# obeychoi0120/wseg

Measured on AMD Instinct MI355X. Metric: training images/sec at B=16x448x448 (contrast_train step), higher is better.
Workload: dtype bf16; 1 GPU; ResNet-38 contrast, synthetic VOC 448x448, B=16/GPU, procedural weights, dropout on, fused HIP loss; global_batch=16, parallelism=dp1, seed=0

## Files before the change

include/wseg_hip.h:

```cpp
#ifndef WSEG_HIP_H
#define WSEG_HIP_H
#include <stddef.h>
#include <stdint.h>
#ifdef __cplusplus
extern "C" {
#endif

#define WSEG_F32 0
#define WSEG_BF16 1
#define WSEG_F32X3 2

int wseg_version(void);
size_t wseg_sizeof_conv_desc(void);
size_t wseg_sizeof_wgrad_desc(void);
const char* wseg_last_error(void);

typedef struct wseg_conv_desc {
  const void* in;  const void* w;  void* out;  void* out2;
  const void* r_pre;  const void* r_post;  const void* mask;
  const float* scale;  const float* shift;  const float* drop;
  int32_t N, IH, IW, IC, ld_in;
  int32_t OH, OW, OC, ld_out, ld_out2;
  int32_t ld_rpre, ld_rpost, ld_mask;
  int32_t KH, KW, stride, dil, pad;
  int32_t mode, epi, dtype;
  int32_t relu_out2;
  int32_t relu_lt;
  int32_t bm_hint;
  int32_t IH2, IW2, OH2, OW2;
  const void* in2;
  int32_t ld_in2, IC2;
  int32_t w_rows;
} wseg_conv_desc;
int wseg_conv_igemm(const wseg_conv_desc* d, void* stream);

typedef struct wseg_wgrad_desc {
  const void* x;  const void* dy;  float* dw;
  int32_t N, IH, IW, IC, ld_x;
  int32_t OH, OW, OC, ld_dy;
  int32_t KH, KW, stride, dil, pad;
  int32_t dtype, split_k;
  int32_t IC_dw, OC_dw;
  int32_t tile_hint;
  int32_t IH2, IW2, OH2, OW2;
  int32_t dw_rot;
} wseg_wgrad_desc;
int wseg_conv_wgrad(const wseg_wgrad_desc* d, void* stream);

#define WSEG_CONV_64x128 1
#define WSEG_CONV_128x128 2
#define WSEG_CONV_224x256 3
#define WSEG_CONV_256x256 4
#define WSEG_CONV_512x128 5
#define WSEG_WGRAD_128x128 6
#define WSEG_WGRAD_256x256 7
typedef struct wseg_launch_plan {
  int32_t family;
  int32_t tile_rows, tile_cols;
  int32_t nwg;
  int32_t perm;
  int32_t tapf;
  int32_t nsplit;
  int32_t unit;
} wseg_launch_plan;
int wseg_conv_plan(const wseg_conv_desc* d, wseg_launch_plan* out);
int wseg_wgrad_plan(const wseg_wgrad_desc* d, wseg_launch_plan* out);

int wseg_conv_bwd_pair(const wseg_conv_desc* dg, const wseg_wgrad_desc* wg, void* stream);
int wseg_conv_bwd_pair_plan(const wseg_conv_desc* dg, const wseg_wgrad_desc* wg, wseg_launch_plan* dg_plan, wseg_launch_plan* wg_plan);

int wseg_pack_weights(const float* master, void* fwd, void* tr, int OC, int T, int IC,
                      int OCp, int ICp, int ic_rot, int dtype, void* stream);
int wseg_copy2d_batch(const void* src, void* dst, const long* table, int npieces, long total_chunks, void* stream);
int wseg_pack_transposed_batch(const float* master, void* out, const long* table, int nlayers, long total_tiles, int dtype, void* stream);
int wseg_pack_transposed_batch_bf16(const void* mirror, void* out, const long* table, int nlayers, long total_tiles, void* stream);
int wseg_dropout_scale(const float* u, float* out, long total, long split_at, float p0, float p1, void* stream);

int wseg_stem_conv(const float* x_nchw, const float* w ,
                   const float* scale, const float* shift, void* raw, void* act,
                   int N, int H, int W, int dtype, void* stream);
int wseg_stem_conv_kc(const float* x, const float* w_kc, const float* scale, const float* shift,
                      void* raw, void* act, int N, int H, int W, int dtype, void* stream);

int wseg_head_split(const void* head, int ld, int c0, float* cam_low, float* cmax, int N, int hw, int dtype, void* stream);
int wseg_cam_gate(const float* cam_low, const float* cmax, float* G, int N, int hw, void* stream);
int wseg_pcm_xs(const float* x_nchw, void* feat, int ld, int c_xs, int c_end, int N, int H, int W, int h, int w, int dtype, void* stream);
int wseg_head_grad_rows(const float* d_fproj, const float* d_cam_low, const void* head, void* d_head, int ld, int N, int hw, int dtype, void* stream);

int wseg_resize_planar_fwd(const float* in, float* out, const float* plane_mul, long planes, int ih, int iw, int oh, int ow, int align,
                           int flip_x, int accumulate, void* stream);
int wseg_resize_planar_bwd(const float* d_out, float* d_in, const float* plane_mul, const float* plane_add, long planes, int ih, int iw, int oh, int ow, int align, int accumulate, void* stream);

int wseg_infer_finish(const float* sum_cam, const float* stats, float alpha, float* norm_cam, unsigned char* pred, int npix, void* stream);

int wseg_l2norm_forward(const void* F, int ldf, float* Fh, float* nrm, long rows, int dtype, void* stream);
int wseg_l2norm_backward(const void* F, int ldf, const float* dFh, const float* nrm, void* dF, int lddf, long rows, int dtype, void* stream);
int wseg_pcm_forward(const float* Fh, const float* G, float* cam_rv, float* den, int N, int hw, void* stream);
int wseg_pcm_backward(const float* Fh, const float* G, const float* d_cam_rv, const float* cam_rv, const float* den,
                      float* DN, float* dFh, int N, int hw, void* stream);
int wseg_pack_x3(const float* src, void* dst, long numel, void* stream);
int wseg_split_bf16(const float* in, void* hi, void* lo, long total, void* stream);
int wseg_to_bf16(const float* in, void* out, long total, void* stream);
int wseg_pcm_forward_bf16(const void* Fb, const void* Gb, float* cam_rv, float* den, int N, int hw, void* stream);
int wseg_pcm_backward_bf16(const void* Fb, const void* Gb, const void* Gl, const float* d_cam_rv, const float* cam_rv, const float* den,
                           float* DN, void* DNb, void* DNl, float* dFh, int N, int hw, void* stream);

size_t wseg_plane_stats_workspace_bytes(long planes);
int wseg_plane_stats(const float* U, float* stats, long planes, int npix, void* workspace, void* stream);
int wseg_up_plane_stats(const float* low, float* stats, long planes, int h, int w, int S, const float* label20 , void* workspace, void* stream);
int wseg_up_rvmin_values(const float* low, const float* label20, float* q, unsigned char* argc, int N, int h, int w, int S, void* stream);
int wseg_up_norm_resize_forward(const float* low, const float* stats, const float* label20, float* out, int N, int h, int w, int S, int OS, void* stream);
int wseg_resize_adjoint_ones(float* wvec, int h, int S, void* stream);
int wseg_up_maps_backward(const float* G, const float* low, const float* stats, const float* label20, const float* plane_bias,
                          const float* wvec_y, const float* wvec_x, const float* q, const unsigned char* argc, const float* res,
                          int k, float coef, float* d_low, int N, int h, int w, int S, int OS, void* stream);
int wseg_cls_loss(const float* stats, const float* label20, float* loss_out, float* plane_bias, int N, int npix, float coef, void* stream);
size_t wseg_select_workspace_bytes(int rows);
int wseg_select_kth(const float* vals, int rows, int n, int k, int largest, int use_abs, int relu_vals, float* res, void* workspace, void* stream);
int wseg_select_finish(const float* res, int rows, int k, int relu_vals, float scale, float* loss_out, void* stream);
int wseg_loss_finish(const float* acc, float er_coef, float* out8, void* stream);
int wseg_er_ecr_prep(const float* c1, const float* c2, const float* r1, const float* r2, float* Gc1, float* Gc2, float* dlt1, float* dlt2,
                     float* er_sum, int N, int npix, float er_coef, void* stream);
int wseg_ecr_backward(const float* dlt, const float* res, float* Gr, int N, int per_row, int k, float coef, void* stream);
int wseg_rows_resize_forward(const void* head, int ld, float* F, int N, int ih, int iw, int oh, int ow, int dtype, void* stream);
int wseg_head_grad_fused(const float* dF, const float* d_cam_low, const void* head, void* d_head, int ld, int N, int ih, int iw, int oh, int ow, int dtype, void* stream);
int wseg_pseudo_label(const float* R, const float* label20, float bg_thr, int* y, float* ncam, int N, int npix, void* stream);
int wseg_proto_candidates(const float* ncam, const float* F, const int* tie_idx, float* cand_val, float* cand_feat, int* cand_const, int N, int npix, int K, void* stream);
int wseg_proto_merge(const float* cand_val, const float* cand_feat, const int* cand_const, float* protos, int world, int K,
                     long rank_stride , void* stream);
int wseg_intra_weights(const int* y, const float* S_own, int ld_s, const float* rkey, const unsigned char* rand_flag, float* w, int P, void* stream);
int wseg_intra_weights_global(const float* rec, float* w, int P, int ranks, int own_rank, float scale, long rank_stride, void* stream);

typedef struct {
  const float* F;
  const float* p_own;
  const float* p_oth;
  const int32_t* y_own;
  const int32_t* y_oth;
  const float* w_intra;
  const float* rkey;
  float* rec;
  float* dF;
} wseg_nce_view;
int wseg_nce_records(const wseg_nce_view* views, int nviews, int P, int split_bf16, void* stream);
int wseg_nce_fused(const wseg_nce_view* views, int nviews, int P, float coef_cross, float coef_intra, float* sums , void* stream);

typedef struct {
  const uint8_t* src; int32_t H, W;
  int32_t rh, rw;
  const int32_t* xb; const int32_t* xk; int32_t xks;
  const int32_t* yb; const int32_t* yk; int32_t yks;
  uint8_t* tmp; uint8_t* img;
  int32_t flip;
  int32_t op[4];
  float factor[4];
  int32_t hue_shift;
  int32_t cont_top, cont_left, img_top, img_left, ch, cw;
  float* out;
} wseg_aug_desc;
size_t wseg_sizeof_aug_desc(void);
int wseg_augment_batch(const wseg_aug_desc* descs_dev, int n, int max_pixels , const float* lut ,
                       int crop, unsigned long long* lum_sums , void* stream);

int wseg_sgd_step(float* params, const float* grads, float* momentum_buf, long numel,
                  const long* seg_begin, const long* seg_end, const float* seg_lr, const float* seg_wd, int nseg,
                  float momentum, float grad_scale, int first_step, void* bf16_mirror, void* stream);

#define WSEG_AFF_MAX_OFFSETS 64
#define WSEG_RW_MAX_PLANE 8192
int wseg_aff_num_offsets(int radius);
int wseg_aff_pairs(const void* feat, int ld, int C, float* aff, int N, int h, int w, int radius, int dtype, void* stream);
int wseg_aff_to_dense(const float* aff, float* dense, int h, int w, int radius, void* stream);
int wseg_rw_prepare(const float* aff, float* wgt, float* rsum, int N, int h, int w, int radius, int beta, void* stream);
int wseg_random_walk(const float* wgt, const float* rsum, const float* v_in, float* v_out, int N, int planes, int h, int w, int radius,
                     int logt, void* stream);
int wseg_rw_pool(const float* cams, const int* src, float bg, float* pooled, int H, int W, int dh, int dw, void* stream);
int wseg_rw_finish(const float* cam_rw, unsigned char* pred, int planes, int dh, int dw, int H, int W, void* stream);

long wseg_aff_loss_workspace_bytes(int N, int h, int w, int radius);
int wseg_aff_loss_forward(const void* feat, int ld, int C, const unsigned char* label, float* aff, void* workspace, float* out7, int N,
                          int h, int w, int radius, int dtype, void* stream);
int wseg_aff_loss_backward(const void* feat, int ld, int C, const unsigned char* label, const float* aff, const float* out7,
                           const float* gscale, float* d_feat, int ld_d, int N, int h, int w, int radius, int dtype, void* stream);

int wseg_elu_backward_rows(const void* g, int ld_g, int g_dtype, const void* y, int ld_y, int y_dtype, const float* gscale, void* dz,
                           int ld_dz, int dz_dtype, long M, int C, void* stream);

#define WSEG_CRF_PIX_ALIGN 128
// ... 21 lines not shown
```

wseg_amd/_lib.py:

```python
import contextlib
import ctypes as C
import os

import torch

_HERE = os.path.dirname(os.path.abspath(__file__))
LIB_PATH = os.environ.get("WSEG_LIB") or os.path.join(_HERE, "libwseg_hip.so")

F32, BF16, F32X3 = 0, 1, 2
PROFILE_WGRAD = None
PROFILE = None
PROFILE_STRIDE = 1
_profile_idx = 0
_profile_phase = 0


def profile_begin_step(step):
    global _profile_idx, _profile_phase
    _profile_idx, _profile_phase = 0, step % max(1, PROFILE_STRIDE)


def _profile_sample():
    global _profile_idx
    i = _profile_idx
# ... 20 lines not shown
    _fields_ = [("x", C.c_void_p), ("dy", C.c_void_p), ("dw", C.c_void_p),
                ("N", C.c_int32), ("IH", C.c_int32), ("IW", C.c_int32), ("IC", C.c_int32), ("ld_x", C.c_int32),
                ("OH", C.c_int32), ("OW", C.c_int32), ("OC", C.c_int32), ("ld_dy", C.c_int32),
                ("KH", C.c_int32), ("KW", C.c_int32), ("stride", C.c_int32), ("dil", C.c_int32), ("pad", C.c_int32),
                ("dtype", C.c_int32), ("split_k", C.c_int32), ("IC_dw", C.c_int32), ("OC_dw", C.c_int32),
                ("tile_hint", C.c_int32),
                ("IH2", C.c_int32), ("IW2", C.c_int32), ("OH2", C.c_int32), ("OW2", C.c_int32), ("dw_rot", C.c_int32)]


def _load():
    if not os.path.exists(LIB_PATH):
        raise ImportError(
            f"{LIB_PATH} not found: build it with `python -c 'import __graft_entry__ as g; g.build()'` "
            "(wseg_amd has no CPU/eager fallback)")
    lib = C.CDLL(LIB_PATH)
    lib.wseg_last_error.restype = C.c_char_p
    lib.wseg_version.restype = C.c_int
    for fn in ("wseg_sizeof_conv_desc", "wseg_sizeof_wgrad_desc", "wseg_select_workspace_bytes", "wseg_plane_stats_workspace_bytes"):
        getattr(lib, fn).restype = C.c_size_t
    if lib.wseg_sizeof_conv_desc() != C.sizeof(ConvDesc) or lib.wseg_sizeof_wgrad_desc() != C.sizeof(WgradDesc):
        raise ImportError(f"{LIB_PATH} was built from another include/wseg_hip.h (descriptor sizes "
                          f"{lib.wseg_sizeof_conv_desc()}/{lib.wseg_sizeof_wgrad_desc()} vs {C.sizeof(ConvDesc)}/{C.sizeof(WgradDesc)}): rebuild it")
    return lib


lib = _load()


def _ptr(t):
    return t.data_ptr() if torch.is_tensor(t) else t


def stream_ptr():
    return torch.cuda.current_stream().cuda_stream


def check(status, what):
    if status != 0:
        raise RuntimeError(f"{what} failed ({status}): {lib.wseg_last_error().decode()}")


def _v(x):
    return C.c_void_p(_ptr(x))


def _s():
    return C.c_void_p(stream_ptr())


def _f(x):
    return C.c_float(x)


def _call(name, *args):
    check(getattr(lib, name)(*args, _s()), name)


def dtype_code(t):
    if t.dtype == torch.float32:
        return F32
    if t.dtype == torch.bfloat16:
        return BF16
    raise TypeError(f"unsupported dtype {t.dtype}")


def _flops_label(kind, *, N, IH, IW, IC, OH, OW, OC, KH, KW, stride=1, dil=1, seg2=None, mode=0, IC2=None, **_):
    oh, ow = (OH, OW) if mode == 0 else (IH, IW)
    pix = N * oh * ow
    if seg2 is not None:
        pix += N * (seg2[2] * seg2[3] if mode == 0 else seg2[0] * seg2[1])
    kin = IC * KH * KW + (IC2 or 0)
    return 2.0 * pix * kin * OC, f"{kind} {IC}{('+%d' % IC2) if IC2 else ''}->{OC} k{KH} s{stride} d{dil} {OH}x{OW}"


@contextlib.contextmanager
def _timed(sink, entry):
    if sink is None:
        yield
        return
    ev0, ev1 = torch.cuda.Event(enable_timing=True), torch.cuda.Event(enable_timing=True)
    ev0.record()
    yield
    ev1.record()
    sink.append((ev0, ev1) + tuple(entry()))


def conv_igemm(inp, w, out=None, out2=None, *, pair_wgrad=None, **kw):
    d = _conv_desc(inp, w, out, out2, **kw)
    ic2 = (d.IC2 or d.IC) if d.in2 else 0
    krow, wrows = d.KH * d.KW * d.IC + ic2, max(d.OC, d.w_rows)
    if w.numel() < wrows * krow:
        raise RuntimeError(f"conv_igemm: weight buffer has {w.numel()} elements, the launch reads {wrows} x {krow}")
    sampled, launch_idx = _profile_sample() if PROFILE is not None else (False, 0)

    def entry():
        kind = "fwd" if d.mode == 0 else ("dgrad+wgrad" if pair_wgrad is not None else "dgrad")
        flops, label = _flops_label(kind, **{**kw, "IC2": ic2})
        wflops = _flops_label("wgrad", **pair_wgrad[3])[0] if pair_wgrad is not None else 0.0
        return flops + wflops, label, launch_idx

    with _timed(PROFILE if sampled else None, entry):
        if pair_wgrad is not None:
            wx, wdy, wdw, wkw = pair_wgrad
            _call("wseg_conv_bwd_pair", C.byref(d), C.byref(_wgrad_desc(wx, wdy, wdw, **wkw)))
        else:
            _call("wseg_conv_igemm", C.byref(d))


def _conv_desc(inp, w, out, out2, *, N, IH, IW, IC, OH, OW, OC, KH, KW, stride=1, dil=1, pad=0,
               mode=0, epi=0, r_pre=None, r_post=None, mask=None, scale=None, shift=None, drop=None,
               ld_in=None, ld_out=None, ld_out2=None, ld_rpre=None, ld_rpost=None, ld_mask=None, relu_out2=1,
               relu_lt=0, bm_hint=0, seg2=None, in2=None, ld_in2=None, IC2=0, dtype=None, w_rows=0):
    d = ConvDesc()
    d.inp, d.w, d.out, d.out2 = _ptr(inp), _ptr(w), _ptr(out), _ptr(out2)
    d.r_pre, d.r_post, d.mask = _ptr(r_pre), _ptr(r_post), _ptr(mask)
    d.scale, d.shift, d.drop = _ptr(scale), _ptr(shift), _ptr(drop)
    d.N, d.IH, d.IW, d.IC, d.ld_in = N, IH, IW, IC, ld_in or IC
    d.OH, d.OW, d.OC, d.ld_out, d.ld_out2 = OH, OW, OC, ld_out or OC, ld_out2 or OC
    d.ld_rpre, d.ld_rpost, d.ld_mask = ld_rpre or OC, ld_rpost or OC, ld_mask or OC
    d.KH, d.KW, d.stride, d.dil, d.pad = KH, KW, stride, dil, pad
    d.mode, d.epi, d.dtype, d.relu_out2, d.relu_lt, d.bm_hint = mode, epi, (dtype_code(inp) if dtype is None else dtype), relu_out2, relu_lt, bm_hint
    if seg2 is not None:
        d.IH2, d.IW2, d.OH2, d.OW2 = seg2
    ic2 = (IC2 or IC) if in2 is not None else 0
    if in2 is not None:
        d.in2, d.IC2, d.ld_in2 = _ptr(in2), IC2, ld_in2 or ic2
    d.w_rows = w_rows
    return d


def _wgrad_desc(x, dy, dw, *, N, IH, IW, IC, OH, OW, OC, KH, KW, stride=1, dil=1, pad=0,
                ld_x=None, ld_dy=None, split_k=0, IC_dw=None, OC_dw=None, tile_hint=0, seg2=None, dtype=None, dw_rot=0):
    d = WgradDesc()
    d.x, d.dy, d.dw = _ptr(x), _ptr(dy), _ptr(dw)
    d.N, d.IH, d.IW, d.IC, d.ld_x = N, IH, IW, IC, ld_x or IC
    d.OH, d.OW, d.OC, d.ld_dy = OH, OW, OC, ld_dy or OC
    d.KH, d.KW, d.stride, d.dil, d.pad = KH, KW, stride, dil, pad
    d.dtype, d.split_k = (dtype_code(x) if dtype is None else dtype), split_k
    d.IC_dw, d.OC_dw, d.tile_hint = IC_dw or IC, OC_dw or OC, tile_hint
    d.dw_rot = dw_rot
    if seg2 is not None:
        d.IH2, d.IW2, d.OH2, d.OW2 = seg2
    assert not torch.is_tensor(dw) or dw.dtype == torch.float32
    return d


def conv_wgrad(x, dy, dw, **kw):
    d = _wgrad_desc(x, dy, dw, **kw)
    with _timed(PROFILE_WGRAD, lambda: _flops_label("wgrad", **kw)):
        _call("wseg_conv_wgrad", C.byref(d))


CONV_64x128, CONV_128x128, CONV_224x256, CONV_256x256, CONV_512x128, WGRAD_128x128, WGRAD_256x256 = range(1, 8)
_ANY = 64


class LaunchPlan(C.Structure):
    _fields_ = [(k, C.c_int32) for k in ("family", "tile_rows", "tile_cols", "nwg", "perm", "tapf", "nsplit", "unit")]

    def __repr__(self):
        return "LaunchPlan(" + ", ".join(f"{k}={getattr(self, k)}" for k, _t in self._fields_) + ")"


def _plan_dtype(t, dtype):
    return dtype if dtype is not None else (dtype_code(t) if torch.is_tensor(t) else BF16)


def conv_plan(inp=_ANY, w=_ANY, out=_ANY, out2=None, *, dtype=None, **kw):
    plan = LaunchPlan()
    check(lib.wseg_conv_plan(C.byref(_conv_desc(inp, w, out, out2, dtype=_plan_dtype(inp, dtype), **kw)), C.byref(plan)), "wseg_conv_plan")
    return plan


def wgrad_plan(x=_ANY, dy=_ANY, dw=_ANY, *, dtype=None, **kw):
    plan = LaunchPlan()
    check(lib.wseg_wgrad_plan(C.byref(_wgrad_desc(x, dy, dw, dtype=_plan_dtype(x, dtype), **kw)), C.byref(plan)), "wseg_wgrad_plan")
    return plan


def conv_pair_plan(wgrad_kw, inp=_ANY, w=_ANY, out=_ANY, out2=None, *, dtype=None, **kw):
    dg, wg = LaunchPlan(), LaunchPlan()
    dtype = _plan_dtype(inp, dtype)
    wdtype = dtype if wgrad_kw.get("dtype") is None else wgrad_kw["dtype"]
    fused = lib.wseg_conv_bwd_pair_plan(C.byref(_conv_desc(inp, w, out, out2, dtype=dtype, **kw)),
                                        C.byref(_wgrad_desc(_ANY, _ANY, _ANY, **{**wgrad_kw, "dtype": wdtype})), C.byref(dg), C.byref(wg))
    if fused < 0:
        check(fused, "wseg_conv_bwd_pair_plan")
    return fused, dg, wg


def pack_weights(master, fwd, tr, OC, T, IC, OCp, ICp, dtype, ic_rot=0):
    _call("wseg_pack_weights", _v(master), _v(fwd), _v(tr), OC, T, IC, OCp, ICp, ic_rot, dtype)


def copy2d_batch(src, dst, table, npieces, total_chunks):
    _call("wseg_copy2d_batch", _v(src), _v(dst), _v(table), npieces, C.c_long(total_chunks))


def pack_transposed_batch(master, out, table, nlayers, total_tiles, dtype):
    _call("wseg_pack_transposed_batch", _v(master), _v(out), _v(table), nlayers, C.c_long(total_tiles), dtype)


def pack_transposed_batch_bf16(mirror, out, table, nlayers, total_tiles):
    _call("wseg_pack_transposed_batch_bf16", _v(mirror), _v(out), _v(table), nlayers, C.c_long(total_tiles))


def dropout_scale(u, out, split_at, p0, p1):
    _call("wseg_dropout_scale", _v(u), _v(out), C.c_long(u.numel()), C.c_long(split_at), _f(p0), _f(p1))


def stem_conv_kc(x, w_kc, scale, shift, raw, act, N, H, W, dtype):
    if w_kc.numel() != 27 * 64 or w_kc.dtype != torch.float32:
        raise RuntimeError("stem_conv_kc: weights must be f32 [27][64]")
    _call("wseg_stem_conv_kc", _v(x), _v(w_kc), _v(scale), _v(shift), _v(raw), _v(act), N, H, W, dtype)


def stem_conv(x, w, scale, shift, raw, act, N, H, W, dtype):
    _call("wseg_stem_conv", _v(x), _v(w), _v(scale), _v(shift), _v(raw), _v(act), N, H, W, dtype)


def head_split(head, ld, c0, cam_low, cmax, N, hw):
    check(lib.wseg_head_split(_v(head), ld, c0, _v(cam_low), _v(cmax), N, hw, dtype_code(head), _s()), "wseg_head_split")


def cam_gate(cam_low, cmax, G, N, hw):
    check(lib.wseg_cam_gate(_v(cam_low), _v(cmax), _v(G), N, hw, _s()), "wseg_cam_gate")


def pcm_xs(x, feat, ld, c_xs, c_end, N, H, W, h, w):
    check(lib.wseg_pcm_xs(_v(x), _v(feat), ld, c_xs, c_end, N, H, W, h, w, dtype_code(feat), _s()), "wseg_pcm_xs")


def head_grad_rows(d_fproj, d_cam_low, head, d_head, ld, N, hw):
    check(lib.wseg_head_grad_rows(_v(d_fproj), _v(d_cam_low), _v(head), _v(d_head), ld, N, hw, dtype_code(head), _s()), "wseg_head_grad_rows")


def resize_planar_fwd(inp, out, planes, ih, iw, oh, ow, align, plane_mul=None, flip_x=False, accumulate=False):
    check(lib.wseg_resize_planar_fwd(_v(inp), _v(out), _v(plane_mul), C.c_long(planes), ih, iw, oh, ow, int(align), int(flip_x), int(accumulate), _s()), "wseg_resize_planar_fwd")


def infer_finish(sum_cam, stats, alpha, norm_cam, pred, npix):
    check(lib.wseg_infer_finish(_v(sum_cam), _v(stats), C.c_float(alpha), _v(norm_cam), _v(pred), npix, _s()), "wseg_infer_finish")


def resize_planar_bwd(d_out, d_in, planes, ih, iw, oh, ow, align, accumulate=False, plane_mul=None, plane_add=None):
    check(lib.wseg_resize_planar_bwd(_v(d_out), _v(d_in), _v(plane_mul), _v(plane_add), C.c_long(planes), ih, iw, oh, ow, int(align), int(accumulate), _s()), "wseg_resize_planar_bwd")


def l2norm_forward(F, ldf, Fh, nrm, rows):
    check(lib.wseg_l2norm_forward(_v(F), ldf, _v(Fh), _v(nrm), C.c_long(rows), dtype_code(F), _s()), "wseg_l2norm_forward")


def l2norm_backward(F, ldf, dFh, nrm, dF, lddf, rows):
    check(lib.wseg_l2norm_backward(_v(F), ldf, _v(dFh), _v(nrm), _v(dF), lddf, C.c_long(rows), dtype_code(F), _s()), "wseg_l2norm_backward")


def pcm_forward(Fh, G, cam_rv, den, N, hw):
    check(lib.wseg_pcm_forward(_v(Fh), _v(G), _v(cam_rv), _v(den), N, hw, _s()), "wseg_pcm_forward")


def pcm_backward(Fh, G, d_cam_rv, cam_rv, den, DN, dFh, N, hw):
    check(lib.wseg_pcm_backward(_v(Fh), _v(G), _v(d_cam_rv), _v(cam_rv), _v(den), _v(DN), _v(dFh), N, hw, _s()), "wseg_pcm_backward")


def sgd_step(params, grads, buf, segs, momentum, grad_scale, first_step, bf16_mirror=None):
    n = len(segs)
    LongArr, FloatArr = C.c_long * n, C.c_float * n
    b = LongArr(*[s[0] for s in segs]); e = LongArr(*[s[1] for s in segs])
    lr = FloatArr(*[s[2] for s in segs]); wd = FloatArr(*[s[3] for s in segs])
    check(lib.wseg_sgd_step(_v(params), _v(grads), _v(buf), C.c_long(params.numel()), b, e, lr, wd, n,
                            C.c_float(momentum), C.c_float(grad_scale), int(first_step), _v(bf16_mirror), _s()), "wseg_sgd_step")


def plane_stats(U, stats, planes, npix):
    ws = torch.empty(int(lib.wseg_plane_stats_workspace_bytes(C.c_long(planes))), device=U.device, dtype=torch.uint8)
    _call("wseg_plane_stats", _v(U), _v(stats), C.c_long(planes), npix, _v(ws))
def cls_loss(stats, label20, loss_out, plane_bias, N, npix, coef): _call("wseg_cls_loss", _v(stats), _v(label20), _v(loss_out), _v(plane_bias), N, npix, _f(coef))
def select_workspace_bytes(rows): return int(lib.wseg_select_workspace_bytes(rows))
def select_kth(vals, rows, n, k, largest, use_abs, relu_vals, res, ws): _call("wseg_select_kth", _v(vals), rows, n, k, int(largest), int(use_abs), int(relu_vals), _v(res), _v(ws))
def loss_finish(acc, er_coef, out8): _call("wseg_loss_finish", _v(acc), _f(er_coef), _v(out8))
def select_finish(res, rows, k, relu_vals, scale, loss_out): _call("wseg_select_finish", _v(res), rows, k, int(relu_vals), _f(scale), _v(loss_out))
def er_ecr_prep(c1, c2, r1, r2, Gc1, Gc2, dlt1, dlt2, er_sum, N, npix, er_coef): _call("wseg_er_ecr_prep", _v(c1), _v(c2), _v(r1), _v(r2), _v(Gc1), _v(Gc2), _v(dlt1), _v(dlt2), _v(er_sum), N, npix, _f(er_coef))
def ecr_backward(dlt, res, Gr, N, per_row, k, coef): _call("wseg_ecr_backward", _v(dlt), _v(res), _v(Gr), N, per_row, k, _f(coef))
def rows_resize_forward(head, ld, F, N, ih, iw, oh, ow): _call("wseg_rows_resize_forward", _v(head), ld, _v(F), N, ih, iw, oh, ow, dtype_code(head))
def head_grad_fused(dF, d_cam_low, head, d_head, ld, N, ih, iw, oh, ow): _call("wseg_head_grad_fused", _v(dF), _v(d_cam_low), _v(head), _v(d_head), ld, N, ih, iw, oh, ow, dtype_code(head))
def pseudo_label(R, label20, bg_thr, y, ncam, N, npix): _call("wseg_pseudo_label", _v(R), _v(label20), _f(bg_thr), _v(y), _v(ncam), N, npix)
def proto_candidates(ncam, F, tie_idx, cand_val, cand_feat, cand_const, N, npix, K): _call("wseg_proto_candidates", _v(ncam), _v(F), _v(tie_idx), _v(cand_val), _v(cand_feat), _v(cand_const), N, npix, K)
def proto_merge(cand_val, cand_feat, cand_const, protos, world, K, rank_stride=0): _call("wseg_proto_merge", _v(cand_val), _v(cand_feat), _v(cand_const), _v(protos), world, K, C.c_long(rank_stride))
def intra_weights(y, S_own, rkey, rand_flag, w, P, ld_s=21): _call("wseg_intra_weights", _v(y), _v(S_own), ld_s, _v(rkey), _v(rand_flag), _v(w), P)
def intra_weights_global(rec, w, P, ranks, own_rank, scale, rank_stride): _call("wseg_intra_weights_global", _v(rec), _v(w), P, ranks, own_rank, _f(scale), C.c_long(rank_stride))


class NceView(C.Structure):
    _fields_ = [("F", C.c_void_p), ("p_own", C.c_void_p), ("p_oth", C.c_void_p), ("y_own", C.c_void_p), ("y_oth", C.c_void_p),
                ("w_intra", C.c_void_p), ("rkey", C.c_void_p), ("rec", C.c_void_p), ("dF", C.c_void_p)]


def _nce_views(views):
    arr = (NceView * len(views))()
    for i, v in enumerate(views):
        for k, _t in NceView._fields_:
            setattr(arr[i], k, _ptr(v.get(k)))
    return arr


def nce_records(views, P, split_bf16=False):
# ... 97 lines not shown
```

wseg_amd/csrc/conv_wgrad_kernels.h:

```cpp
#include <stdlib.h>
#include <algorithm>
#include <type_traits>
#pragma once
#include "common.h"

#ifdef WSEG_PROBES
#define WG_DIAG(a) ((a).diag)
#else
#define WG_DIAG(a) 0
#endif

namespace wseg_wg {
namespace {

template <int OFF>
__device__ __forceinline__ void tr_read(bf16x4& dst, unsigned addr) {
  asm volatile("ds_read_b64_tr_b16 %0, %1 offset:%2" : "=v"(dst) : "v"(addr), "n"(OFF));
}

struct Args {
  wseg_wgrad_desc d;
  int M, taps, nto, nti, ntiles;
  int pix_per_split;
  int nsplit, nwg;
// ... 462 lines not shown
      const long jump = (long)(b_begin - y_m) * d.ld_dy * 2;
#pragma unroll
      for (int k = 0; k < 2; ++k) ybase[k] += jump;
      y_m = b_begin; y_lim = t.m_end;
    }
    char* to = dst(buf, h);
    const int rem = WG_DIAG(a) == 5 ? 0 : y_lim - y_m;
#pragma unroll
    for (int k = 0; k < 2; ++k) {
      const char* p = rry[k][h] < rem ? ybase[k] + h * 256 : zsrc;
      glds16(p, to + k * 8192);
    }
    if (h == 1) {
#pragma unroll
      for (int k = 0; k < 2; ++k) ybase[k] += ystep;
      y_m += PK; ++ty_idx;
    }
  }
};

template <int UNIT>
__device__ __forceinline__ void conv_wgrad_pipe_tile(const Args& a, char* smem, const int bid) {
  constexpr int BO = 256, BI = 256;
  constexpr int HALF = 16384, ROWB = 256;
  const wseg_wgrad_desc& d = a.d;
  const int tid = threadIdx.x, lane = tid & 63;
  const int wid = __builtin_amdgcn_readfirstlane(tid >> 6);
  const WgTile wt = wg_tile_of<BO, BI>(a, bid);
  if (wt.m_begin >= wt.m_end) return;
  std::conditional_t<UNIT != 0, StageUnit, StageGeneral> st(a, wt, smem, tid, wid);

  const int wr = wid >> 2, wc = wid & 3;
  const int fcol = lane & 15, fk = lane >> 4;
  const int q = (lane & 15) >> 2, p = lane & 3;
  const unsigned lds0 = (unsigned)(size_t)(__attribute__((address_space(3))) char*)smem;

  f32x4 acc[8][4];
#pragma unroll
  for (int i = 0; i < 8; ++i)
#pragma unroll
    for (int j = 0; j < 4; ++j) acc[i][j] = (f32x4){0.f, 0.f, 0.f, 0.f};

  const int nt = st.ntiles();
  st.issue_y(0, 0); st.issue_y(1, 0);
  st.prepare_x(); st.issue_x(0, 0); st.issue_x(1, 0);
  if (nt > 1) { st.prepare_x(); st.issue_x(0, 1); st.issue_x(1, 1); asm volatile("s_waitcnt vmcnt(4)" ::: "memory"); }
  else asm volatile("s_waitcnt vmcnt(0)" ::: "memory");
  asm volatile("s_barrier" ::: "memory");

  bf16x4 va[2][2][4], vb0[2][2][2], vb1[2][2][2];
  bf16x8 af[2][4], b0[2][2], b1[2][2];
#define PACK_A()                                                                                                \
  _Pragma("unroll") for (int ks = 0; ks < 2; ++ks) _Pragma("unroll") for (int i = 0; i < 4; ++i)               \
    af[ks][i] = __builtin_shufflevector(va[ks][0][i], va[ks][1][i], 0, 1, 2, 3, 4, 5, 6, 7);
#define PACK_B(BF, VB)                                                                                          \
  _Pragma("unroll") for (int ks = 0; ks < 2; ++ks) _Pragma("unroll") for (int j = 0; j < 2; ++j)               \
    BF[ks][j] = __builtin_shufflevector(VB[ks][0][j], VB[ks][1][j], 0, 1, 2, 3, 4, 5, 6, 7);
#define WAIT_LDS() do { asm volatile("s_waitcnt lgkmcnt(0)" ::: "memory"); __builtin_amdgcn_sched_barrier(0); } while (0)
#define MFMA_Q(HA, HB, BF)                                                                                      \
  do {                                                                                                          \
    __builtin_amdgcn_s_setprio(1);                                                                              \
    _Pragma("unroll") for (int ks = 0; ks < 2; ++ks) _Pragma("unroll") for (int i = 0; i < 4; ++i)             \
      _Pragma("unroll") for (int j = 0; j < 2; ++j)                                                            \
        acc[(HA) * 4 + i][(HB) * 2 + j] =                                                                       \
            __builtin_amdgcn_mfma_f32_16x16x32_bf16(af[ks][i], BF[ks][j], acc[(HA) * 4 + i][(HB) * 2 + j], 0, 0, 0); \
    __builtin_amdgcn_s_setprio(0);                                                                              \
  } while (0)

  {
    unsigned LTA[8], LTB[4];
    {
      const unsigned s_ = swz32(fk * 8 + q);
      const unsigned rowterm = lds0 + (unsigned)(fk * 8 + q) * ROWB + (unsigned)p * 8;
#pragma unroll
      for (int t = 0; t < 8; ++t) LTA[t] = rowterm + (((unsigned)t ^ s_) << 5) + (unsigned)(wr * 2) * HALF;
#pragma unroll
      for (int t = 0; t < 4; ++t) LTB[t] = rowterm + (((unsigned)((wc & 1) * 4 + t) ^ s_) << 5) + (unsigned)((2 + (wc >> 1)) * 2) * HALF;
    }
    auto ktile = [&](auto BC, int u) {
      constexpr int b = decltype(BC)::value;
      constexpr int BO = b * HALF;
#pragma unroll
      for (int i = 0; i < 4; ++i) {
        tr_read<BO + 0>(va[0][0][i], LTA[i]); tr_read<BO + 1024>(va[0][1][i], LTA[i]);
        tr_read<BO + 8192>(va[1][0][i], LTA[i]); tr_read<BO + 9216>(va[1][1][i], LTA[i]);
      }
#pragma unroll
      for (int j = 0; j < 2; ++j) {
        tr_read<BO + 0>(vb0[0][0][j], LTB[j]); tr_read<BO + 1024>(vb0[0][1][j], LTB[j]);
        tr_read<BO + 8192>(vb0[1][0][j], LTB[j]); tr_read<BO + 9216>(vb0[1][1][j], LTB[j]);
        tr_read<BO + 0>(vb1[0][0][j], LTB[2 + j]); tr_read<BO + 1024>(vb1[0][1][j], LTB[2 + j]);
        tr_read<BO + 8192>(vb1[1][0][j], LTB[2 + j]); tr_read<BO + 9216>(vb1[1][1][j], LTB[2 + j]);
      }
      if (u + 1 < nt && WG_DIAG(a) != 6) { st.issue_y(0, b ^ 1); st.issue_y(1, b ^ 1); }
      WAIT_LDS();
      PACK_A() PACK_B(b0, vb0) PACK_B(b1, vb1)
      MFMA_Q(0, 0, b0);
      MFMA_Q(0, 1, b1);
      asm volatile("s_barrier" ::: "memory");
#pragma unroll
      for (int i = 0; i < 4; ++i) {
        tr_read<BO + 0>(va[0][0][i], LTA[4 + i]); tr_read<BO + 1024>(va[0][1][i], LTA[4 + i]);
        tr_read<BO + 8192>(va[1][0][i], LTA[4 + i]); tr_read<BO + 9216>(va[1][1][i], LTA[4 + i]);
      }
      if (u + 2 < nt) { if (WG_DIAG(a) != 6) { st.prepare_x(); st.issue_x(0, b); st.issue_x(1, b); } asm volatile("s_waitcnt vmcnt(4)" ::: "memory"); }
      else asm volatile("s_waitcnt vmcnt(0)" ::: "memory");
      WAIT_LDS();
      PACK_A()
      MFMA_Q(1, 1, b1);
      MFMA_Q(1, 0, b0);
      asm volatile("s_barrier" ::: "memory");
    };
    int u = 0;
    for (; u + 1 < nt; u += 2) {
      ktile(std::integral_constant<int, 0>{}, u);
      ktile(std::integral_constant<int, 1>{}, u + 1);
    }
    if (u < nt) ktile(std::integral_constant<int, 0>{}, u);
  }
#undef PACK_A
#undef PACK_B
#undef WAIT_LDS
#undef MFMA_Q
  __syncthreads();

  constexpr int WLD = 64 + 4;
  float* wimg = reinterpret_cast<float*>(smem) + wid * (16 * WLD);
  const size_t row_stride = (size_t)a.taps * d.IC_dw;
  const int ic = wt.ic0 + wc * 64 + lane;
  const bool ic_ok = ic < d.IC_dw;
#pragma unroll
  for (int i = 0; i < 8; ++i) {
#pragma unroll
    for (int j = 0; j < 4; ++j)
#pragma unroll
      for (int e = 0; e < 4; ++e) wimg[(fk * 4 + e) * WLD + j * 16 + fcol] = acc[i][j][e];
    asm volatile("s_waitcnt lgkmcnt(0)" ::: "memory");
    const int oc_base = wt.oc0 + wr * 128 + i * 16;
#pragma unroll
    for (int r = 0; r < 16; ++r) {
      const int oc = oc_base + r;
      if (ic_ok && oc < d.OC_dw) atomicAdd(&d.dw[(size_t)oc * row_stride + (size_t)wt.tap * d.IC_dw + ic], wimg[r * WLD + lane]);
    }
    asm volatile("s_waitcnt lgkmcnt(0)" ::: "memory");
  }
}

template <int UNIT>
__global__ __launch_bounds__(512, 2) void conv_wgrad_pipe_kernel(const Args a) {
  __shared__ __attribute__((aligned(16))) char smem[2 * 4 * 16384];
  conv_wgrad_pipe_tile<UNIT>(a, smem, blockIdx.x);
}

struct Plan { Args a; bool pipe; bool unit; };
static int wgrad_plan(const wseg_wgrad_desc* d, Plan& pl) {
  Args& a = pl.a;
  WSEG_CHECK(d && d->x && d->dy && d->dw, "conv_wgrad: null pointer");
  WSEG_CHECK(d->dtype == WSEG_F32 || d->dtype == WSEG_BF16 || d->dtype == WSEG_F32X3, "conv_wgrad: bad dtype");
  WSEG_CHECK(d->IC % 8 == 0 && d->OC % 8 == 0 && d->ld_x % 8 == 0 && d->ld_dy % 8 == 0,
             "conv_wgrad: IC/OC/ld must be multiples of 8 (IC=%d OC=%d ld_x=%d ld_dy=%d)", d->IC, d->OC, d->ld_x, d->ld_dy);
  WSEG_CHECK(d->ld_x >= d->IC && d->ld_dy >= d->OC, "conv_wgrad: leading dims too small");
  WSEG_CHECK(d->IC_dw > 0 && d->IC_dw <= d->IC && d->OC_dw > 0 && d->OC_dw <= d->OC, "conv_wgrad: bad dw extents");
  WSEG_CHECK(d->dw_rot >= 0 && d->dw_rot < d->IC_dw, "conv_wgrad: dw_rot=%d must lie in [0, IC_dw)", d->dw_rot);
  WSEG_CHECK(d->N > 0 && d->OH > 0 && d->OW > 0 && d->IH > 0 && d->IW > 0 && d->stride >= 1 && d->dil >= 1, "conv_wgrad: bad shape");
  const long M = (long)d->N * d->OH * d->OW + (long)d->N * d->OH2 * d->OW2;
  WSEG_CHECK(d->OH2 >= 0 && (d->OH2 == 0 || (d->OW2 > 0 && d->IH2 > 0 && d->IW2 > 0)), "conv_wgrad: bad second segment");
  WSEG_CHECK(M < (1L << 31), "conv_wgrad: too many pixels");
  const bool big = d->dtype == WSEG_BF16 && d->OC >= 256 && d->IC >= 256 && d->tile_hint != 128 &&
                   (M >= 16384 || d->tile_hint == 256);
  const int BO = big ? 256 : 128, BI = BO;
  a.d = *d;
  a.M = (int)M;
  a.taps = d->KH * d->KW;
  a.nto = (d->OC + BO - 1) / BO;
  a.nti = (d->IC + BI - 1) / BI;
  a.ntiles = a.nto * a.nti * a.taps;
  const int pk = d->dtype == WSEG_BF16 ? 64 : 32;
  int split = d->split_k;
  if (split <= 0) {
    const long slots = big ? 256 : 512;
    const double epi = big ? 28.0 : 10.0;
    const int max_split = (int)std::max(1L, std::min(64L, M / (pk * 8)));
    double best = 1e30;
    split = 1;
    for (int sp = 1; sp <= max_split; ++sp) {
      const long blocks = (long)a.ntiles * sp;
      const long rounds = (blocks + slots - 1) / slots;
      const double steps = (double)((M + sp - 1) / sp + pk - 1) / pk;
      const double cost = rounds * (steps + epi) * (1.0 + 0.002 * sp);
      if (cost < best) { best = cost; split = sp; }
    }
  }
  long pps = (M + split - 1) / split;
  pps = (pps + pk - 1) / pk * pk;
  a.pix_per_split = (int)pps;
  split = (int)((M + pps - 1) / pps);
  a.nsplit = split;
  a.nwg = a.ntiles * split;
  a.q64_1 = 64 / d->OW; a.r64_1 = 64 % d->OW;
  a.q64_2 = d->OH2 ? 64 / d->OW2 : 0; a.r64_2 = d->OH2 ? 64 % d->OW2 : 0;
  a.simple_adv = (a.q64_1 + 1 <= d->OH) && (d->OH2 == 0 || a.q64_2 + 1 <= d->OH2);
#ifdef WSEG_PROBES
  static const int diag = getenv("WSEG_WGRAD_DIAG") ? atoi(getenv("WSEG_WGRAD_DIAG")) : 0;
  a.diag = diag;
#else
  a.diag = 0;
#endif
  pl.unit = a.simple_adv && d->stride == 1 && d->IH == d->OH && d->IW == d->OW && (d->OH2 == 0 || (d->IH2 == d->OH2 && d->IW2 == d->OW2));
  pl.pipe = big;
  WSEG_CHECK(d->dw_rot == 0 || !pl.pipe, "conv_wgrad: dw_rot is supported by the 128-tile kernel only");
  return 0;
}
static void wgrad_plan_report(const Plan& pl, wseg_launch_plan* out) {
  const int t = pl.pipe ? 256 : 128;
  *out = wseg_launch_plan{pl.pipe ? WSEG_WGRAD_256x256 : WSEG_WGRAD_128x128, t, t, pl.a.nwg, 0, 0, pl.a.nsplit, pl.pipe && pl.unit};
}
}
}
```

wseg_amd/engine.py:

```python
import threading
import weakref
from typing import NamedTuple

import torch

from . import arch
from . import _lib as L

HEAD_LD = 192
FEAT_LD = 256
AFF_FEAT_C = 448
AFF_FEAT_SLICES = {"f8_3": (0, 64), "f8_4": (64, 192), "f8_5": (192, 448)}


CONTRAST_FLAT_HEAD_ORDER = ("fc_proj", "fc8", "f8_3", "f8_4", "f9")
DT_OF = {"bf16": L.BF16, "fp32": L.F32, "bf16x3": L.F32X3}


def _cdt(dt):
    return L.F32X3 if dt == L.F32X3 else None


class Conv(NamedTuple):
    name: str
# ... 564 lines not shown
            ps = _Pass(N, dev, DT_OF[self.net.precision], P)
        M = ps.rows_of(dims)
        C = AFF_FEAT_C

        def conv(inp, name, out, cin, cout):
            ps.conv(Conv(name, cin, cout, 1, 1, 1, dims, dims), inp, out, epi=3, ld_out=C)

        feat = ps.E(M, C)
        for name, inp in (("f8_3", conv4), ("f8_4", conv5), ("f8_5", t)):
            (cout, cin), c0 = arch.AFF_HEAD_CONVS[name], AFF_FEAT_SLICES[name][0]
            conv(inp, name, feat.view(-1)[c0:] if c0 else feat, cin, cout)
        f9 = ps.E(M, C)
        conv(feat, "f9", f9, C, C)
        return feat, f9

    def aff_head_wt(self, device):
        dt = DT_OF[self.net.precision]
        with self.lock:
            P = self._ensure_packs(device, dt)
            if "f9" not in P["wt"]:
                pdt = L.F32 if dt == L.F32X3 else dt
                for nm, off, n, (ci, _t, co) in self.aff_head_wt_specs():
                    wt = torch.empty(ci, 1, co, device=device, dtype=L.TORCH_DTYPE[dt])
                    L.pack_weights(self.flat_w[off:off + n], None, wt, co, 1, ci, co, ci, pdt)
                    P["wt"][nm] = self._x3(wt) if dt == L.F32X3 else wt
        self._join_late_packs(device)
        return P

    def aff_head_wt_specs(self):
        return [(nm, *self.offsets[nm], (ci, 1, co)) for nm, (co, ci) in self.net.HEAD_CONVS.items()]

    def run_forward(self, xs, save, lowres=False, prefix=None):
        net = self.net
        V = len(xs)
        assert V in (1, 2)
        dev = xs[0].device
        dt = DT_OF[net.precision]
        P = self.ensure_packs(dev, dt)
        N = xs[0].shape[0]
        assert all(x.shape[0] == N for x in xs)
        masks = self._masks(N, V, dev)
        S = {"masks": masks, "dims": {}, "N": N, "V": V, "dt": dt, "xs": xs, "lowres": lowres}
        if prefix is None:
            prefix = self._run_blocks(xs, None, 0, arch.N_FROZEN_BLOCKS, save and self.capture_ctx, S if (save and self.capture_ctx) else None)
        assert prefix["N"] == N and prefix["V"] == V and prefix["dt"] == dt and prefix["in_dims"] == [tuple(x.shape[2:]) for x in xs], \
            "run_forward: the prefix was computed for another batch shape / precision"
        S["dims"].update(prefix["sdims"])
        st = self._run_blocks(xs, prefix, arch.N_FROZEN_BLOCKS, len(arch.BLOCKS), save, S)
        t, dims, conv4, conv5 = st["t"], st["dims"], st["conv4"], st["conv5"]
        ps = _Pass(N, dev, dt, P)
        E, conv = ps.E, ps.conv

        def head_conv(nm, cin, cout):
            return Conv(nm, cin, cout, 1, 1, 1, dims, dims)

        fea = t
        self._join_late_packs(dev)
        M = ps.rows_of(dims)
        offs = ps.offs_of(dims)
        head = E(M, HEAD_LD)
        conv(head_conv("head", 4096, HEAD_LD), fea, head, relu_lt=128, w_rows=256)
        feat = E(M, FEAT_LD)
        conv(head_conv("f8_3", 512, 64), conv4, feat, epi=2, ld_out=FEAT_LD)
        conv(head_conv("f8_4", 1024, 128), conv5, feat.view(-1)[64:], epi=2, ld_out=FEAT_LD)
        G = torch.empty(M, 32, device=dev, dtype=torch.float32)
        views = []
        for x, off, (h, w) in zip(xs, offs, dims):
            hw = h * w
            cam_low = torch.empty(N, 21, h, w, device=dev, dtype=torch.float32)
            cmax = torch.empty(N, 21, device=dev, dtype=torch.float32)
            L.head_split(head[off:], HEAD_LD, 128, cam_low, cmax, N, hw)
            L.cam_gate(cam_low, cmax, G[off:], N, hw)
            L.pcm_xs(x, feat[off:], FEAT_LD, 192, FEAT_LD, N, x.shape[2], x.shape[3], h, w)
            views.append(dict(h=h, w=w, H=x.shape[2], W=x.shape[3], off=off, rows=N * hw, cam_low=cam_low))
        Fm = E(M, 192)
        conv(head_conv("f9", FEAT_LD, 192), feat, Fm)
        Fh = torch.empty(M, 192, device=dev, dtype=torch.float32)
        nrm = torch.empty(M, device=dev, dtype=torch.float32)
        L.l2norm_forward(Fm, 192, Fh, nrm, M)
        Fb = Gb = Gl = None
        if dt == L.BF16:
            Fb = torch.empty(M, 192, device=dev, dtype=torch.bfloat16)
            Gb = torch.empty(M, 32, device=dev, dtype=torch.bfloat16)
            L.to_bf16(Fh, Fb)
            if save:
                Gl = torch.empty(M, 32, device=dev, dtype=torch.bfloat16)
                L.split_bf16(G, Gb, Gl)
            else:
                L.to_bf16(G, Gb)
        outs = []
        for vw, x in zip(views, xs):
            h, w, off, hw = vw["h"], vw["w"], vw["off"], vw["h"] * vw["w"]
            rvd = torch.empty(N, 21, h, w, device=dev, dtype=torch.float32)
            den = torch.empty(N, hw, device=dev, dtype=torch.float32)
            if dt == L.BF16:
                L.pcm_forward_bf16(Fb[off:], Gb[off:], rvd, den, N, hw)
            else:
                L.pcm_forward(Fh[off:], G[off:], rvd, den, N, hw)
            head_v = head[off:off + N * hw].view(N, h, w, HEAD_LD)
            f_proj = head_v[..., :128].permute(0, 3, 1, 2)
            if lowres:
                outs.append((vw["cam_low"], rvd, f_proj, head_v))
            else:
                H, W = vw["H"], vw["W"]
                cam = torch.empty(N, 21, H, W, device=dev, dtype=torch.float32)
                cam_rv = torch.empty(N, 21, H, W, device=dev, dtype=torch.float32)
                L.resize_planar_fwd(vw["cam_low"], cam, N * 21, h, w, H, W, True)
                L.resize_planar_fwd(rvd, cam_rv, N * 21, h, w, H, W, True)
                outs.append((cam, cam_rv, f_proj.float() if dt == L.BF16 else f_proj, rvd))
            vw.update(rvd=(rvd if lowres else rvd.clone()) if save else None, den=den)
        if save and self.capture_ctx:
            self.last_ctx = S
        if save:
            S.update(fea=fea, head=head, G=G, feat=feat, Fm=Fm, Fh=Fh, Fb=Fb, Gb=Gb, Gl=Gl, nrm=nrm, conv4=conv4, conv5=conv5,
                     views=views, hdims=dims, M=M)
        return outs, S

    def run_backward(self, S, grads, d_head_rows=None):
        self.finish_packs()
        P = self.packs
        dt = S["dt"]
        N, M = S["N"], S["M"]
        hdims = S["hdims"]
        dev = S["fea"].device
        masks = S["masks"]
        self.attach_grads()
        ps = _Pass(N, dev, dt, P)
        E, rows_of = ps.E, ps.rows_of

        def trainable(nm):
            return self.conv_param(nm).requires_grad

        def head_conv(nm, cin, cout):
            return Conv(nm, cin, cout, 1, 1, 1, hdims, hdims)

        main = torch.cuda.current_stream(dev)
        pcm_join = [None]

        planes = {}

        def split(t_):
            key = (t_.data_ptr(), t_.numel())
            if key not in planes:
                hi, lo = torch.empty(t_.shape, device=dev, dtype=torch.bfloat16), torch.empty(t_.shape, device=dev, dtype=torch.bfloat16)
                L.split_bf16(t_, hi, lo)
                planes[key] = (hi, lo, t_)
            return planes[key][:2]

        def wgrad(c, x, dy, **kw):
            if not trainable(c.name):
                return
            dw = self.grad_slice(c.name)
            args = dict(c.wgrad_kw(N), dtype=_cdt(dt), **kw)
            if dt == L.F32X3 and c.cin >= 256 and c.cout >= 256 and not kw and x.is_contiguous() and dy.is_contiguous() \
                    and x.shape[1] == c.cin and dy.shape[1] == c.cout:
                (xh, xl), (dh, dl) = split(x), split(dy)
                args["dtype"] = None
                L.conv_wgrad(xl, dh, dw, **args)
                L.conv_wgrad(xh, dl, dw, **args)
                L.conv_wgrad(xh, dh, dw, **args)
            else:
                L.conv_wgrad(x, dy, dw, **args)

        def block_done(nm):
            if self.block_done_hook is not None:
                if pcm_join[0] is not None:
                    main.wait_stream(pcm_join[0])
                    pcm_join[0] = None
                self.block_done_hook(nm)

        def dgrad(c, dy, out, pair=None, **kw):
            pw = None
            if pair is not None and dt == L.BF16 and trainable(pair[0].name):
                pc, px, pdy = pair
                pw = (px, pdy, self.grad_slice(pc.name), dict(pc.wgrad_kw(N), dtype=_cdt(dt)))
            L.conv_igemm(dy, P["wt"][c.name], out, None, dtype=_cdt(dt), pair_wgrad=pw, **c.dgrad_kw(N), **kw)
            if pair is not None and pw is None:
                wgrad(*pair)

        d_cam_low, d_rvd = [], []
        for vw, (g_cam, g_cam_rv, g_fproj, g_rvd) in zip(S["views"], grads):
            h, w, H, W = vw["h"], vw["w"], vw["H"], vw["W"]
            if S["lowres"]:
                d_cam_low.append(g_cam)
                d_rvd.append(g_cam_rv)
                continue
            dc = None
            if g_cam is not None:
                dc = torch.empty(N, 21, h, w, device=dev, dtype=torch.float32)
                L.resize_planar_bwd(g_cam.contiguous().float(), dc, N * 21, h, w, H, W, True)
            dr = None
            if g_cam_rv is not None:
                dr = torch.empty(N, 21, h, w, device=dev, dtype=torch.float32)
                L.resize_planar_bwd(g_cam_rv.contiguous().float(), dr, N * 21, h, w, H, W, True)
            if g_rvd is not None:
                dr = g_rvd.contiguous().float() if dr is None else dr + g_rvd
            d_cam_low.append(dc)
            d_rvd.append(dr)
        pcm_stream = None
        if any(d is not None for d in d_rvd):
            pcm_stream = self.stream("pcm", dev)
            pcm_stream.wait_stream(main)
            with torch.cuda.stream(pcm_stream):
                DN = torch.empty(M, 32, device=dev, dtype=torch.float32)
                dFh = torch.zeros(M, 192, device=dev, dtype=torch.float32)
                DNb = torch.empty(M, 32, device=dev, dtype=torch.bfloat16) if S["Fb"] is not None else None
                DNl = torch.empty(M, 32, device=dev, dtype=torch.bfloat16) if S["Fb"] is not None else None
                for vw, dr in zip(S["views"], d_rvd):
                    if dr is None:
                        continue
                    off, hw = vw["off"], vw["h"] * vw["w"]
                    if S["Fb"] is not None:
                        L.pcm_backward_bf16(S["Fb"][off:], S["Gb"][off:], S["Gl"][off:], dr.contiguous(), vw["rvd"], vw["den"], DN[off:], DNb[off:],
                                            DNl[off:], dFh[off:], N, hw)
                    else:
                        L.pcm_backward(S["Fh"][off:], S["G"][off:], dr.contiguous(), vw["rvd"], vw["den"], DN[off:], dFh[off:], N, hw)
                dF = E(M, 192)
                L.l2norm_backward(S["Fm"], 192, dFh, S["nrm"], dF, 192, M)
                wgrad(head_conv("f9", FEAT_LD, 192), S["feat"], dF, IC_dw=195, dw_rot=3)
                if trainable("f8_3") or trainable("f8_4"):
                    d_feat = E(M, FEAT_LD)
                    dgrad(head_conv("f9", FEAT_LD, 192), dF, d_feat, epi=1, mask=S["feat"])
                    wgrad(head_conv("f8_3", 512, 64), S["conv4"], d_feat, ld_dy=FEAT_LD)
                    wgrad(head_conv("f8_4", 1024, 128), S["conv5"], d_feat.view(-1)[64:], ld_dy=FEAT_LD)
        pcm_join[0] = pcm_stream
        if d_head_rows is None:
            if all(dc is None for dc in d_cam_low) and all(g[2] is None for g in grads):
                if pcm_stream is not None:
                    main.wait_stream(pcm_stream)
                return
            d_head_rows = E(M, HEAD_LD)
            for vw, dc, g in zip(S["views"], d_cam_low, grads):
                off, hw = vw["off"], vw["h"] * vw["w"]
                gf = g[2].contiguous().float() if g[2] is not None else None
                L.head_grad_rows(gf, dc.contiguous() if dc is not None else None, S["head"][off:], d_head_rows[off:], HEAD_LD, N, hw)
        chead = head_conv("head", 4096, HEAD_LD)
        if trainable("fc_proj") or trainable("fc8"):
            L.conv_wgrad(S["fea"], d_head_rows, self.grad_slice("fc_proj", 149 * 4096), OC_dw=149, dtype=_cdt(dt), **chead.wgrad_kw(N))
        s7, _ = P["bn"]["bn7"]
        D = E(M, 4096)
        dgrad(chead, d_head_rows, D, epi=1, scale=s7, drop=masks["dropout7"] if masks else None, mask=S["fea"])
        for i in range(len(arch.BLOCKS) - 1, -1, -1):
            b = arch.BLOCKS[i]
            name, kind, cin, mid, cout, stride, fd, d, p = b
            if name in arch.FROZEN_BLOCKS:
                break
            same = arch.block_same_shape(b)
            din, dout = S["dims"][name]
            Mi = rows_of(din)
            Mo = rows_of(dout)
            sv = S[name]
            sa, _ = P["bn"][name + ".bn_branch2a"]
            first_trainable = name == "b3"
            c1 = Conv(name + ".conv_branch1", cin, cout, 1, stride, 1, din, dout)
            if kind == "res":
                s1, _ = P["bn"][name + ".bn_branch2b1"]
                c2a = Conv(name + ".conv_branch2a", cin, mid, 3, stride, fd, din, dout)
                c2b1 = Conv(name + ".conv_branch2b1", mid, cout, 3, 1, d, dout, dout)
                du = E(Mo, mid)
                dgrad(c2b1, D, du, epi=1, scale=s1, mask=sv["v"], pair=(c2b1, sv["v"], D))
                fused_skip = (name + ".skip_fused") in P["wt"] and not first_trainable
                if not (same and not first_trainable):
                    wgrad(c2a, sv["t"], du)
                if not same and not fused_skip:
                    wgrad(c1, sv["t"], D)
                if first_trainable:
                    block_done(name)
                    break
                Din = E(Mi, cin)
                if same:
                    dgrad(c2a, du, Din, epi=1, scale=sa, mask=sv["t"], r_post=D, pair=(c2a, sv["t"], du))
                elif fused_skip:
                    dgrad(c2a._replace(name=name + ".skip_fused"), du, Din, in2=D, IC2=cout, epi=1, scale=sa, mask=sv["t"], pair=(c1, sv["t"], D))
                else:
                    tmp = E(Mi, cin)
                    dgrad(c1, D, tmp)
                    dgrad(c2a, du, Din, epi=1, scale=sa, mask=sv["t"], r_pre=tmp)
                D = Din
                block_done(name)
            else:
                c4, c2 = cout // 4, cout // 2
                s1, _ = P["bn"][name + ".bn_branch2b1"]
                s2, _ = P["bn"][name + ".bn_branch2b2"]
                d1 = masks[name + ".dropout_2b1"] if masks else None
                d2 = masks[name + ".dropout_2b2"] if masks else None
                c2a = Conv(name + ".conv_branch2a", cin, c4, 1, stride, 1, din, dout)
                c2b1 = Conv(name + ".conv_branch2b1", c4, c2, 3, 1, d, dout, dout)
                c2b2 = Conv(name + ".conv_branch2b2", c2, cout, 1, 1, 1, dout, dout)
                du2 = E(Mo, c2)
                dgrad(c2b2, D, du2, epi=1, scale=s2, drop=d2, mask=sv["v2"], pair=(c2b2, sv["v2"], D))
                du1 = E(Mo, c4)
                dgrad(c2b1, du2, du1, epi=1, scale=s1, drop=d1, mask=sv["v1"], pair=(c2b1, sv["v1"], du2))
                wgrad(c2a, sv["t"], du1)
                Din = E(Mi, cin)
                if (name + ".skip_fused") in P["wt"]:
                    dgrad(Conv(name + ".skip_fused", cin, cout, 1, 1, 1, din, dout), D, Din, epi=1, scale=sa, mask=sv["t"], in2=du1, IC2=c4,
                          pair=(c1, sv["t"], D))
                else:
                    tmp = E(Mi, cin)
                    dgrad(c1, D, tmp, pair=(c1, sv["t"], D))
                    dgrad(c2a, du1, Din, epi=1, scale=sa, mask=sv["t"], r_pre=tmp)
                D = Din
                block_done(name)
        planes.clear()
        if pcm_join[0] is not None:
            main.wait_stream(pcm_join[0])


class _NetFunction(torch.autograd.Function):
    @staticmethod
    def forward(ctx, x, anchor, eng, lowres):
        outs, S = eng.run_forward([x], save=True, lowres=lowres)
        ctx.eng, ctx.S = eng, S
        ctx.set_materialize_grads(False)
        if lowres:
            ctx.mark_non_differentiable(outs[0][3])
        return outs[0]

    @staticmethod
    def backward(ctx, g0, g1, g2, g3):
        S = ctx.S
        ctx.eng.run_backward(S, [(g0, g1, g2, None if S["lowres"] else g3)])
        ctx.S = None
        return None, None, None, None
```

Before: 469.3 images/sec.

## Pick wgrad tile size and split-K from a per-kernel timing cost model

Adds a time-based cost model for weight-gradient launches on narrow bf16 convolutions (IC or OC below 256). It evaluates both the 128-tile and 256-tile pipelined kernels with per-step and epilogue time constants and picks the cheaper tile along with its split-K. It also allows larger split counts when there are few tiles, so the GPU stays filled. The engine now passes this hint for all bf16 wgrad calls, including fc_proj. The risk is that the hardcoded constants mispredict and pick slower configurations, and that larger splits add more atomic-add traffic.

```diff
diff --git a/include/wseg_hip.h b/include/wseg_hip.h
--- a/include/wseg_hip.h
+++ b/include/wseg_hip.h
@@ -34,6 +34,8 @@
 } wseg_conv_desc;
 int wseg_conv_igemm(const wseg_conv_desc* d, void* stream);
 
+#define WSEG_TILE_BY_TIME 1
+#define WSEG_TILE_PIPE 257
 typedef struct wseg_wgrad_desc {
   const void* x;  const void* dy;  float* dw;
   int32_t N, IH, IW, IC, ld_x;
diff --git a/wseg_amd/_lib.py b/wseg_amd/_lib.py
--- a/wseg_amd/_lib.py
+++ b/wseg_amd/_lib.py
@@ -196,6 +196,7 @@
 
 
 CONV_64x128, CONV_128x128, CONV_224x256, CONV_256x256, CONV_512x128, WGRAD_128x128, WGRAD_256x256 = range(1, 8)
+TILE_BY_TIME, TILE_PIPE = 1, 257
 _ANY = 64
 
 
diff --git a/wseg_amd/csrc/conv_wgrad_kernels.h b/wseg_amd/csrc/conv_wgrad_kernels.h
--- a/wseg_amd/csrc/conv_wgrad_kernels.h
+++ b/wseg_amd/csrc/conv_wgrad_kernels.h
@@ -638,6 +638,12 @@
   conv_wgrad_pipe_tile<UNIT>(a, smem, blockIdx.x);
 }
 
+struct WgradTimes { double kstep_us, epi_us; };
+static constexpr WgradTimes kPipeUnit = {1.45, 12.0};
+static constexpr WgradTimes kPipeGeneral = {1.75, 12.0};
+static constexpr WgradTimes kTile128Alone = {1.56, 17.0};
+static constexpr WgradTimes kTile128Shared = {1.94, 24.0};
+
 struct Plan { Args a; bool pipe; bool unit; };
 static int wgrad_plan(const wseg_wgrad_desc* d, Plan& pl) {
   Args& a = pl.a;
@@ -652,31 +658,56 @@
   const long M = (long)d->N * d->OH * d->OW + (long)d->N * d->OH2 * d->OW2;
   WSEG_CHECK(d->OH2 >= 0 && (d->OH2 == 0 || (d->OW2 > 0 && d->IH2 > 0 && d->IW2 > 0)), "conv_wgrad: bad second segment");
   WSEG_CHECK(M < (1L << 31), "conv_wgrad: too many pixels");
-  const bool big = d->dtype == WSEG_BF16 && d->OC >= 256 && d->IC >= 256 && d->tile_hint != 128 &&
-                   (M >= 16384 || d->tile_hint == 256);
+  const int hint = d->tile_hint;
+  const bool pipe_able = d->dtype == WSEG_BF16 && d->dw_rot == 0;
+  const bool wide = d->dtype == WSEG_BF16 && d->OC >= 256 && d->IC >= 256;
+  const bool narrow = d->dtype == WSEG_BF16 && !wide;
+  const bool by_time = hint == WSEG_TILE_BY_TIME && narrow && pipe_able && M >= 16384;
+  const bool cover = (hint == WSEG_TILE_BY_TIME || hint == WSEG_TILE_PIPE) && narrow;
+  const bool unit_geo = d->stride == 1 && d->IH == d->OH && d->IW == d->OW && (d->OH2 == 0 || (d->IH2 == d->OH2 && d->IW2 == d->OW2));
+  const int pk = d->dtype == WSEG_BF16 ? 64 : 32;
+  const int taps = d->KH * d->KW;
+  auto pick_split = [&](bool pipe, int& split_out) {
+    const int B = pipe ? 256 : 128;
+    const long ntiles = (long)((d->OC + B - 1) / B) * ((d->IC + B - 1) / B) * taps;
+    const long slots = pipe ? 256 : 512;
+    const double epi = pipe ? 28.0 : 10.0;
+    long max_split = std::max(1L, std::min(64L, M / (pk * 8)));
+    if (cover && ntiles < 8) max_split = std::max(max_split, std::min((slots + ntiles - 1) / ntiles, M / (pk * 4)));
+    double best = 1e30;
+    int split = 1;
+    for (int sp = 1; sp <= max_split; ++sp) {
+      const long blocks = ntiles * sp;
+      const long rounds = (blocks + slots - 1) / slots;
+      const double steps = (double)((M + sp - 1) / sp + pk - 1) / pk;
+      double cost = rounds * (steps + epi) * (1.0 + 0.002 * sp);
+      if (cover) {
+        const WgradTimes& t = pipe ? (unit_geo ? kPipeUnit : kPipeGeneral) : (blocks <= 256 ? kTile128Alone : kTile128Shared);
+        cost = rounds * (steps * t.kstep_us + t.epi_us) * (1.0 + 0.002 * sp);
+      }
+      if (cost < best) { best = cost; split = sp; }
+    }
+    split_out = split;
+    return best;
+  };
+  bool big = hint == WSEG_TILE_PIPE ? pipe_able
+                                    : wide && hint != 128 && (M >= 16384 || hint == 256);
+  int split = d->split_k;
+  if (by_time) {
+    int sp128, sp256;
+    const double t128 = pick_split(false, sp128), t256 = pick_split(true, sp256);
+    big = t256 < t128;
+    if (split <= 0) split = big ? sp256 : sp128;
+  } else if (split <= 0) {
+    pick_split(big, split);
+  }
   const int BO = big ? 256 : 128, BI = BO;
   a.d = *d;
   a.M = (int)M;
-  a.taps = d->KH * d->KW;
+  a.taps = taps;
   a.nto = (d->OC + BO - 1) / BO;
   a.nti = (d->IC + BI - 1) / BI;
   a.ntiles = a.nto * a.nti * a.taps;
-  const int pk = d->dtype == WSEG_BF16 ? 64 : 32;
-  int split = d->split_k;
-  if (split <= 0) {
-    const long slots = big ? 256 : 512;
-    const double epi = big ? 28.0 : 10.0;
-    const int max_split = (int)std::max(1L, std::min(64L, M / (pk * 8)));
-    double best = 1e30;
-    split = 1;
-    for (int sp = 1; sp <= max_split; ++sp) {
-      const long blocks = (long)a.ntiles * sp;
-      const long rounds = (blocks + slots - 1) / slots;
-      const double steps = (double)((M + sp - 1) / sp + pk - 1) / pk;
-      const double cost = rounds * (steps + epi) * (1.0 + 0.002 * sp);
-      if (cost < best) { best = cost; split = sp; }
-    }
-  }
   long pps = (M + split - 1) / split;
   pps = (pps + pk - 1) / pk * pk;
   a.pix_per_split = (int)pps;
@@ -692,7 +723,7 @@
 #else
   a.diag = 0;
 #endif
-  pl.unit = a.simple_adv && d->stride == 1 && d->IH == d->OH && d->IW == d->OW && (d->OH2 == 0 || (d->IH2 == d->OH2 && d->IW2 == d->OW2));
+  pl.unit = a.simple_adv && unit_geo;
   pl.pipe = big;
   WSEG_CHECK(d->dw_rot == 0 || !pl.pipe, "conv_wgrad: dw_rot is supported by the 128-tile kernel only");
   return 0;
diff --git a/wseg_amd/engine.py b/wseg_amd/engine.py
--- a/wseg_amd/engine.py
+++ b/wseg_amd/engine.py
@@ -740,6 +740,8 @@
                 return
             dw = self.grad_slice(c.name)
             args = dict(c.wgrad_kw(N), dtype=_cdt(dt), **kw)
+            if dt == L.BF16:
+                args["tile_hint"] = L.TILE_BY_TIME
             if dt == L.F32X3 and c.cin >= 256 and c.cout >= 256 and not kw and x.is_contiguous() and dy.is_contiguous() \
                     and x.shape[1] == c.cin and dy.shape[1] == c.cout:
                 (xh, xl), (dh, dl) = split(x), split(dy)
@@ -824,7 +826,8 @@
                 L.head_grad_rows(gf, dc.contiguous() if dc is not None else None, S["head"][off:], d_head_rows[off:], HEAD_LD, N, hw)
         chead = head_conv("head", 4096, HEAD_LD)
         if trainable("fc_proj") or trainable("fc8"):
-            L.conv_wgrad(S["fea"], d_head_rows, self.grad_slice("fc_proj", 149 * 4096), OC_dw=149, dtype=_cdt(dt), **chead.wgrad_kw(N))
+            L.conv_wgrad(S["fea"], d_head_rows, self.grad_slice("fc_proj", 149 * 4096), OC_dw=149, dtype=_cdt(dt),
+                         tile_hint=L.TILE_BY_TIME if dt == L.BF16 else 0, **chead.wgrad_kw(N))
         s7, _ = P["bn"]["bn7"]
         D = E(M, 4096)
         dgrad(chead, d_head_rows, D, epi=1, scale=s7, drop=masks["dropout7"] if masks else None, mask=S["fea"])
```

Result: no change. 471.5 images/sec (median of 6 runs) (+0.5%).
